# GadGadGad/Convolutional-KAN-for-Image-Classification

Hardware: AMD Instinct MI355X
Metric: images/sec fwd+bwd KAN-VGG11 3x32x32 bs=256/GPU (higher is better)
Workload: dtype f32

## Files before the change

### convolutional-kan-for-image-classification_amd/_lib.py

```python
from __future__ import annotations

import ctypes as C
import os
from typing import Optional

_HERE = os.path.dirname(os.path.abspath(__file__))
LIB_PATH = os.environ.get("KANCONV_LIB") or os.path.join(_HERE, "libkanconv.so")

KAN_MAX_PLANES = 16
KAN_MAX_TABLE = 32
KAN_FP_WORDS = 192
BASIS_BSPLINE, BASIS_RBF, BASIS_CHEBY, BASIS_POLY, BASIS_FOURIER, BASIS_RELU, BASIS_GRAM = 0, 1, 2, 3, 4, 5, 6
ACT_NONE, ACT_IDENTITY, ACT_GELU, ACT_SILU, ACT_RELU, ACT_TANH, ACT_SIGMOID, ACT_GELU_TANH = -1, 0, 1, 2, 3, 4, 5, 6


class KanGeom(C.Structure):
    _fields_ = [(n, C.c_int) for n in ("B", "C", "H", "W", "O", "Ho", "Wo", "kh", "kw", "sh", "sw", "ph", "pw", "dh", "dw", "groups")] + \
               [("x_bstride", C.c_longlong), ("y_bstride", C.c_longlong)]


class KanBasis(C.Structure):
    _fields_ = [("kind", C.c_int), ("n_basis", C.c_int), ("order", C.c_int), ("act", C.c_int),
                ("p0", C.c_float), ("p1", C.c_float), ("table", C.c_float * KAN_MAX_TABLE), ("chan_table", C.c_void_p)]


class KanPlan(C.Structure):
    _fields_ = [(n, C.c_int) for n in ("P", "K", "IPC", "KC", "Kpad", "Opad", "fwd_splits", "bwd_data_splits", "bwd_weight_splits",
                                          "fwd_target", "bwd_data_target", "bwd_weight_target", "x_pm_wanted", "dz_pm_wanted", "bwd_weight_expanded", "row_blocks", "e_pm_wanted", "fwd_expanded", "fwd_halo", "bwd_weight_halo",
# ... 11 lines not shown


class KanWavGeom(C.Structure):
    _fields_ = [(n, C.c_int) for n in ("B", "C", "H", "W", "O", "Ho", "Wo", "kh", "kw", "sh", "sw", "ph", "pw", "dh", "dw", "wavelet")] + \
               [("x_bstride", C.c_longlong), ("u_bstride", C.c_longlong)]


WAVELETS = {"mexican_hat": 0, "morlet": 1, "dog": 2, "meyer": 3, "shannon": 4}

_P, _I, _LL, _F, _D = C.c_void_p, C.c_int, C.c_longlong, C.c_float, C.c_double
_GP, _BP = C.POINTER(KanGeom), C.POINTER(KanBasis)
SIGNATURES = {
    "kan_version": (C.c_char_p, []),
    "kan_last_error": (C.c_char_p, []),
    "kan_plan": (_I, [_GP, _BP, C.POINTER(KanPlan)]),
    "kan_pack_weights": (_I, [_P, _P, _P, _P, _GP, _BP, _P]),
    "kan_pack_cacheable": (_I, [_GP, _BP]),
    "kan_pack_weights_cached": (_I, [_P, _P, _P, _P, _GP, _BP, _P, _I, _I, _I, _P]),
    "kan_conv_fwd": (_I, [_P, _P, _P, _P, _GP, _BP, _P, _P]),
    "kan_position_major": (_I, [_P, _P, _I, _I, _I, _LL, _P]),
    "kan_conv_bwd_data": (_I, [_P, _P, _P, _P, _P, _P, _GP, _BP, _P, _P]),
    "kan_conv_bwd_data_params": (_I, [_P, _P, _P, _P, _P, _P, _P, _GP, _BP, _P, _P]),
    "kan_conv_bwd_weight": (_I, [_P, _P, _P, _P, _GP, _BP, _P, _P, _P]),
    "kan_position_major_expanded": (_I, [_P, _P, _GP, _BP, _P]),
    "kan_conv_fwd_expanded": (_I, [_P, _P, _P, _GP, _BP, _P]),
    "kan_conv_bwd_weight_expanded": (_I, [_P, _P, _P, _GP, _BP, _P]),
    "kan_unpack_wgrad": (_I, [_P, _P, _P, _GP, _BP, _P]),
    "kan_slab_reduce": (_I, [_P, _I, _LL, _P, _I, _I, _I, _LL, _P]),
    "kan_instnorm_prelu_fwd": (_I, [_P, _I, _LL, _P, _P, _P, _P, _P, _P, _P, _I, _I, _I, _LL, _F, _I, _P]),
    "kan_instnorm_prelu_bwd": (_I, [_P, _P, _P, _P, _P, _P, _P, _P, _P, _P, _P, _I, _I, _I, _LL, _I, _P]),
# ... 48 lines not shown
```

### convolutional-kan-for-image-classification_amd/csrc/kan_internal.h

```cpp
#pragma once
#include <type_traits>
#include "kanconv.h"

int kan_fail_msg(const char* fmt, const char* a);
int kan_raise_lds_limit(const void* kernel, int bytes);

enum : int {
    FAST_GENERIC = 0,
    FAST_BSPLINE_SILU = 1,
    FAST_BSPLINE_GELU = 2,
    FAST_RBF8 = 3,
    FAST_CHEBY5 = 4,
    FAST_CHEBY4 = 5,
    FAST_POLY4 = 6,
    FAST_POLY3 = 7,
    FAST_RBF5 = 8,
    FAST_RELU8 = 9,
    FAST_GRAM4 = 10,
    FAST_POLY1 = 11,
    FAST_LAST = 11
};
enum : unsigned {
    ON_TAP_MAJOR = 1u << 0,
    ON_BIG_TILES = 1u << 1,
// ... 91 lines not shown

enum class Route { TAP_MAJOR, DW, BAND, HALO, EXPANDED };

struct FwdCfg { int TO, TP, tiles_o, tiles_p, chunks, splits, slots; };
struct BdCfg { int CH, tiles_c, tiles_p, n_ob, Opad32, chunks, splits; };
struct BwCfg { int TR, TO, tiles_r, tiles_o, chunks, splits, slots; };
struct BwHaloCfg { int R, nimg, spb, n_bands, tiles_r, tiles_o, splits, bands_per_split; };

struct ConvPlan {
    KanPlan pub;
    int fast;
    Route fwd, bwd_data, bwd_weight;
    bool pm_fwd, pm_bwd_data, pm_bwd_weight;
    bool rowblk_bwd_data;
    bool quad_fwd;
    bool pmdma_xcd, pm_lpt, pm_xcd;
    FwdCfg fc;
    BdCfg bd;
    BwCfg bw;
    BwHaloCfg bwh;
    KanBandCfg band;
};
int plan_conv(const KanGeom* g, const KanBasis* b, ConvPlan* cp);

int live_taps_out(const KanGeom* g, int hw);
int live_taps_in(const KanGeom* g, int hw);
int live_positions_for_tap(const KanGeom* g, int tap);
int balance_tiles(const int* weight, int n, unsigned short* idx);
```

### convolutional-kan-for-image-classification_amd/csrc/kan_plan.hip

```cpp
#include <hip/hip_runtime.h>
#include <cstdio>
#include <cstdlib>
#include <cstring>
#include "kanconv.h"
#include "kan_device.h"
#include "kan_common.h"
#include "kan_internal.h"

namespace {

int fail(const char* msg) { return kan_fail_msg("%s", msg); }

int check(const KanGeom* g, const KanBasis* b) {
    if (!g || !b) return fail("null geometry/basis");
    if (g->groups < 0 || g->groups > 65535) return fail("groups out of range");
    if (g->B <= 0 || g->C <= 0 || g->O <= 0 || g->H <= 0 || g->W <= 0 || g->Ho <= 0 || g->Wo <= 0) return fail("non-positive dimension");
    if (g->kh <= 0 || g->kw <= 0 || g->sh <= 0 || g->sw <= 0 || g->dh <= 0 || g->dw <= 0 || g->ph < 0 || g->pw < 0) return fail("bad conv parameters");
    if (g->kh > 255 || g->kw > 255 || g->C > 65535) return fail("kernel size / channel count out of supported range");
    if ((g->H + 2 * g->ph - g->dh * (g->kh - 1) - 1) / g->sh + 1 != g->Ho || (g->W + 2 * g->pw - g->dw * (g->kw - 1) - 1) / g->sw + 1 != g->Wo)
        return fail("Ho/Wo inconsistent with H/W, kernel, stride, padding, dilation");
    if ((long long)g->B * g->Ho * g->Wo >= (1ll << 31) || (long long)g->B * g->H * g->W >= (1ll << 31)) return fail("pixel count exceeds int32");
    if ((long long)g->B * g->x_bstride * 4 >= (1ll << 31) || (long long)g->B * g->y_bstride * 4 >= (1ll << 31))
        return fail("activation tensors must be smaller than 2 GiB (32-bit buffer offsets)");
    if (g->x_bstride < (long long)ngroups(g) * g->C * g->H * g->W || g->y_bstride < (long long)ngroups(g) * g->O * g->Ho * g->Wo)
// ... 324 lines not shown
    pl->bwd_weight_slab_elems = (long long)G * pl->K * pl->Opad;
    const bool big = big_tiles(f, *pl);
    c.fc = fwd_cfg(g, *pl, big, c.pm_fwd, halo);
    c.bw = bw_cfg(g, *pl, big, c.pm_bwd_weight);
    if (halo_bw) c.bwh = bw_halo_cfg(g, *pl);
    pl->fwd_splits = band ? c.band.fwd_splits : c.fc.splits;
    pl->bwd_data_splits = c.bd.splits;
    pl->bwd_weight_splits = halo_bw ? c.bwh.splits : c.bw.splits;
    if (band_bw) {
        pl->bwd_weight_splits = c.band.bw_splits;
        pl->bwd_weight_slab_elems = (long long)G * pl->Kpad * pl->Opad;
    }
    pl->fwd_target = pl->bwd_data_target = pl->bwd_weight_target = 0;
    const bool rowblk_fwd = halo && g->H == 4 && g->W == 4 && c.fc.TO == 256;
    c.quad_fwd = rowblk_fwd && g->B % 32 == 0 && !tuning_off("KAN_QUAD_FWD");
    if (dw) {
        pl->fwd_splits = pl->bwd_data_splits = 1;
        pl->bwd_weight_splits = dw_weight_chunks(g);
        pl->bwd_data_weight_bytes = pl->packed_weight_bytes;
        c.pm_fwd = c.pm_bwd_data = c.pm_bwd_weight = false;
    }
    if (c.pm_fwd) {
        LiveClass cls[16]; const int plane = g->Ho * g->Wo;
        const long long tiles_per_pos = (long long)ceil_div(g->B, c.fc.TP) * c.fc.tiles_o * G;
        for (int hw = 0; hw < plane; ++hw) cls[hw] = LiveClass{tiles_per_pos, live_taps_out(g, hw) * ceil_div(g->C, pl->IPC)};
        pl->fwd_target = pick_target_steps(cls, plane, 8, 4.0 * g->B * g->O * g->Ho * g->Wo * G, &pl->fwd_splits, c.fc.slots);
    }
    if (c.pm_bwd_weight) {
        LiveClass cw[32];
        const long long tiles_per_tap = (long long)ceil_div((long long)g->C * pl->P, c.bw.TR) * c.bw.tiles_o * G;
// ... 23 lines not shown
```

### convolutional-kan-for-image-classification_amd/csrc/kanconv.hip

```cpp
#include <hip/hip_runtime.h>
#include <cstdio>
#include <cstdlib>
#include <cstring>
#include <cmath>
#include <cstdint>
#include <mutex>
#include <type_traits>
#include <vector>
#include "kanconv.h"
#include "kan_device.h"

#include "kan_common.h"
#include "kan_internal.h"

namespace {


thread_local char g_err[512] = "";
int fail(const char* fmt, const char* a = "") {
    snprintf(g_err, sizeof(g_err), fmt, a);
    return -1;
}
}
int kan_fail_msg(const char* fmt, const char* a) { return fail(fmt, a); }
// ... 406 lines not shown
#define LDS_READ3H(r0, r1, r2, addrA, addrB, oA0, oA1, oB)                                                               \
    asm volatile("ds_read_b32 %0, %3 offset:%5\n\tds_read_b32 %1, %3 offset:%6\n\tds_read_b32 %2, %4 offset:%7"         \
                 : "=&v"(r0), "=&v"(r1), "=&v"(r2) : "v"(addrA), "v"(addrB), "n"(oA0), "n"(oA1), "n"(oB) : "memory")
#define LDS_WAIT3(r0, r1, r2, N) asm volatile("s_waitcnt lgkmcnt(" #N ")" : "+v"(r0), "+v"(r1), "+v"(r2) :: "memory")

template <int FAST, int WO, int W, int R, int NIMG, int QUAD = 0>
__global__ __launch_bounds__(WO * 2 * 64, ((WO > 2 && !(R * W == 16 && NIMG * W == 32)) ? 2 : 4)) void k_conv_fwd_halo(
    const float* __restrict__ x, const float* __restrict__ wp, float* __restrict__ z, DevGeom g, DevBasis bs, int Opad,
    int n_pairs, int pairs_per_split, long long slab_elems, unsigned x_bytes, int tiles_o) {
    constexpr int TO = WO * 64, TP = 128, NT = WO * 2 * 64, NW = WO * 2, P = fast_planes(FAST), KC = 2 * P, T = 9;
    constexpr int KIND = fast_kind(FAST);
    constexpr int HW_ = QUAD ? 3 : W + 2, HIMG = QUAD ? 9 : (R + 2) * HW_, HALO = (QUAD ? 32 : NIMG) * HIMG;
    constexpr int RPI = 256 / TO, NQ = (KC + RPI - 1) / RPI;
    static_assert(NIMG * R * W == TP && HALO % 2 == 0, "tile shape");
    static_assert(!QUAD || (R * W == 16 && NIMG * W == 32 && WO == 4), "the quadrant order is a variant of the row-block tile");
    constexpr bool ROWBLK = (R * W == 16 && NIMG * W == 32 && WO == 4) && !QUAD;
    constexpr int HPAD = QUAD ? 4 : 0;
    __shared__ __attribute__((aligned(16))) float sW[2 * KC * TO];
    __shared__ float sH_[2 * P * HALO + 2 * HPAD];
    float* const sH = sH_ + HPAD;
    __shared__ float sTab[KAN_MAX_TABLE];
    __shared__ float sDump[NT];

    const int tid = threadIdx.x, lane = tid & 63;
    const int wave = __builtin_amdgcn_readfirstlane(tid >> 6);
    const int w_o = (ROWBLK || QUAD) ? (wave & 3) : (wave >> 1), w_p = (ROWBLK || QUAD) ? (wave >> 2) : (wave & 1);
    const int HoWo = g.Ho * g.Wo, HW = g.H * g.W, Mtot = g.B * HoWo;
    const BlockId blk = xcd_block_order(true);
    const int grp = blk.y / tiles_o;
    const int qh = (blk.x >> 1) & 1, qw = blk.x & 1;
    const int px_tile0 = blk.x * TP, o_tile0 = (blk.y - grp * tiles_o) * TO;
    x += (size_t)grp * g.C * HW;
    z += (size_t)grp * g.O * HoWo;
    wp += (size_t)grp * n_pairs * (T * KC) * Opad;

    if (tid < KAN_MAX_TABLE) sTab[tid] = bs.tab[tid];
    for (int i = tid; i < 2 * P * HALO + 2 * HPAD; i += NT) sH_[i] = 0.f;

    const int b0 = QUAD ? (blk.x >> 2) * 32 : px_tile0 / HoWo, h0 = QUAD ? 0 : (px_tile0 - b0 * HoWo) / W;
    constexpr int NCELL = 2 * HALO, CPT = (NCELL + NT - 1) / NT;
    int c_src[CPT], c_dst[CPT], c_ch[CPT]; unsigned c_ok = 0;
#pragma unroll
    for (int k = 0; k < CPT; ++k) {
        const int idx = tid + k * NT;
        const int ch = idx / HALO, cell = idx - ch * HALO;
        const int img = cell / HIMG, rc = cell - img * HIMG, hr = rc / HW_, hc = rc - hr * HW_;
        const int b = b0 + img, h = QUAD ? qh + hr : h0 - 1 + hr, w = QUAD ? qw + hc : hc - 1;
        const bool ok = idx < NCELL && b < g.B && (unsigned)h < (unsigned)g.H && (unsigned)w < (unsigned)W;
        c_src[k] = b * (int)g.xbs + ch * HW + h * W + w;
        c_dst[k] = ch * (P * HALO) + cell;
        c_ch[k] = ch;
        c_ok |= (ok ? 1u : 0u) << k;
    }
    const kan_rsrc x_rs = make_rsrc(x, x_bytes);
// ... 59 lines not shown
        __syncthreads();
#pragma unroll
        for (int k = 0; k < CPT; ++k)
            if ((c_ok >> k) & 1u) stage_unit<KIND, FAST>(bs, sTab, true, xv[k], xv[k], sH + c_dst[k], HALO, sDump + tid, 2 * cp + c_ch[k]);
#pragma unroll 1
        for (int tap = 0; tap < T; ++tap) {
            asm volatile("s_waitcnt vmcnt(0)" ::: "memory");
            __syncthreads();
            const int nxt = cp * T + tap + 1;
            if (nxt < cp1 * T) issue_w(nxt, buf ^ 1);
            if (tap == 4 && cp + 1 < cp1) load_pair(cp + 1);
            const int r = tap / 3, t = tap - r * 3;
            const unsigned sh = (unsigned)(((r - 1) * HW_ + (t - 1)) * 4);
            const unsigned aw = lds_addr(sW + buf * (KC * TO) + kh2 * TO + ao), ab0 = vb[0] + sh, ab1 = vb[1] + sh;
            float fa[2][2], fb[2][2];
            const int dead = !ROWBLK ? -1 : (r == 0 && w_p == 0) ? 0 : (r == 2 && w_p == 1) ? 1 : -1;
            const bool live0 = QUAD ? ((q_live[0] >> tap) & 1u) != 0 : dead != 0, live1 = QUAD ? ((q_live[1] >> tap) & 1u) != 0 : dead != 1;
            LDS_READ4H(fa[0][0], fa[0][1], fb[0][0], fb[0][1], aw, ab0, ab1, 0, 32 * 4, 0);
#pragma unroll
            for (int kk = 0; kk < P; ++kk) {
                const int c_ = kk & 1, n_ = c_ ^ 1;
                if (kk + 1 < P) {
                    LDS_READ4H(fa[n_][0], fa[n_][1], fb[n_][0], fb[n_][1], aw, ab0, ab1, (2 * (kk + 1)) * TO * 4, (2 * (kk + 1)) * TO * 4 + 128,
                               (kk + 1) * HALO * 4);
                    LDS_WAIT4(fa[c_][0], fa[c_][1], fb[c_][0], fb[c_][1], 4);
                } else {
                    LDS_WAIT4(fa[c_][0], fa[c_][1], fb[c_][0], fb[c_][1], 0);
                }
                if (!(ROWBLK || QUAD) || live0) {
                    acc[0][0] = MFMA32(fa[c_][0], fb[c_][0], acc[0][0]);
                    acc[1][0] = MFMA32(fa[c_][1], fb[c_][0], acc[1][0]);
// ... 13 lines not shown
#pragma unroll
        for (int mi = 0; mi < 2; ++mi) {
#pragma unroll
            for (int r = 0; r < 16; ++r) {
                const int o = o_tile0 + w_o * 64 + mi * 32 + mfma_row(r, lane);
                if (o < g.O) *reinterpret_cast<float2*>(zb + (size_t)o * HoWo) = make_float2(acc[mi][0][r], acc[mi][1][r]);
            }
        }
        return;
    }
#pragma unroll
    for (int ni = 0; ni < 2; ++ni) {
        int px = px_tile0 + w_p * 64 + ni * 32 + (lane & 31);
        if (ROWBLK) {
            const int l = lane & 31;
            px = px_tile0 + (l >> 2) * (R * W) + (w_p * 2 + ni) * W + (l & 3);
        }
        if (px >= Mtot) continue;
        const int b = px / HoWo, hw = px - b * HoWo;
        float* zb = zs + (size_t)b * g.ybs + hw;
#pragma unroll
        for (int mi = 0; mi < 2; ++mi) {
#pragma unroll
            for (int r = 0; r < 16; ++r) {
                const int o = o_tile0 + w_o * 64 + mi * 32 + mfma_row(r, lane);
                if (o < g.O) zb[(size_t)o * HoWo] = acc[mi][ni][r];
            }
        }
    }
}

// ... 9 lines not shown
#pragma unroll
            for (int i = 0; i < M / 2; ++i) {
                if (i < h) {
                    const float keep = up ? v[h + i] : v[i], send = up ? v[i] : v[h + i];
                    v[i] = keep + __shfl_xor(send, off, 64);
                }
            }
            base += up ? h : 0;
            m = h;
        } else {
            v[0] += __shfl_xor(v[0], off, 64);
        }
    }
    idx = base; tot = v[0];
}

template <int KIND, int FAST, int RB = 0>
__global__ __launch_bounds__(256, 4) void k_conv_bwd_data(
    const float* __restrict__ dz, const float* __restrict__ x, const float* __restrict__ xn, const float* __restrict__ wd,
    float* __restrict__ dx, float* __restrict__ dxn, DevGeom g, DevBasis bs, int CH, int n_ct, int n_ob, int Opad16,
    int n_chunks, int chunks_per_split, long long slab_elems, unsigned dz_bytes, TilePerm perm, float* __restrict__ dpar) {
    constexpr int TP = 128, KD = 16, NT = 256;
    __shared__ __attribute__((aligned(16))) float smem[2 * 2 * KD * 128];
    __shared__ float sTab[KAN_MAX_TABLE];

    const int tid = threadIdx.x, lane = tid & 63;
    const int wave = __builtin_amdgcn_readfirstlane(tid >> 6);
    const int w_r = wave >> 1, w_p = wave & 1;
    const int HoWo = g.Ho * g.Wo, HW = g.H * g.W, P = bs.P;
    const int Min = g.B * HW;
    const BlockId blk = xcd_block_order(false);
    const int grp = blk.y / n_ct;
    const int px_tile0 = (perm.n ? (int)perm.idx[blk.x] : blk.x) * TP, ct = blk.y - grp * n_ct;
    const int ncol = n_ct * 128;
    const int pxl = (wave & 1) * 64 + lane, ol0 = wave >> 1;
    const bool idle_rows = (ct * 2 + w_r) * CH >= g.C;
    {
        const size_t xo = (size_t)grp * g.C * HW;
        x += xo; xn += xo; dx += xo; if (dxn) dxn += xo;
        dz += (size_t)grp * g.O * HoWo * (g.pix_major ? g.B : 1);
        wd += (size_t)grp * (g.kh * g.kw) * Opad16 * ncol;
    }

    if (tid < KAN_MAX_TABLE) sTab[tid] = bs.tab[tid];
    const int my_px = px_tile0 + (RB ? ((pxl >> 2) & 7) * 16 + (pxl >> 5) * 4 + (pxl & 3) : pxl);
    const bool pv = my_px < Min;
    int pb, ph_, pw_;
    {
        int hw;
        if (g.pix_major) { hw = my_px / g.B; pb = my_px - hw * g.B; }
        else { pb = my_px / HW; hw = my_px - pb * HW; }
        ph_ = hw / g.W; pw_ = hw - ph_ * g.W;
    }
    const kan_rsrc dz_rs = make_rsrc(dz, dz_bytes);
    const unsigned dz_img = g.pix_major ? (unsigned)pb : (unsigned)pb * (unsigned)g.ybs;
    const unsigned zstride = g.pix_major ? (unsigned)g.B : 1u;
    const int wv = wave;

    int cur_tap = -1; unsigned base = KAN_OOB;
    const unsigned wlane = (unsigned)((lane >> 5) * ncol + (lane & 31) * 4) * 4u;
// ... 65 lines not shown
        } else {
#pragma unroll
            for (int n = 0; n < 8; ++n)
                __builtin_amdgcn_raw_ptr_buffer_load_lds(dz_rs, (__attribute__((address_space(3))) void*)(dG + (ol0 + 2 * n) * TP), 4,
                                                         (int)baseA, (int)(soA + (unsigned)(2 * n) * row_bytes), 0, 0);
        }
        const int tapA = mixed ? t : 3 + t, tapB = 6 + t;
#pragma unroll
        for (int j = 0; j < 2; ++j) {
            const int blk2 = j * 4 + wv;
            const int row = mixed ? ((blk2 < 4 ? tapA : tapB) * Opad16 + o0 + (blk2 & 3) * 2) : (tapA * Opad16 + o0 + blk2 * 2);
            glds16((const float*)((const char*)(wd + (size_t)row * ncol + ct * 128) + wlane), dW + blk2 * 256);
        }
    };

    f32x16 acc[2][2];
#pragma unroll
    for (int a = 0; a < 2; ++a)
#pragma unroll
        for (int b = 0; b < 2; ++b)
#pragma unroll
            for (int r = 0; r < 16; ++r) acc[a][b][r] = 0.f;

    int ch0 = blk.z * chunks_per_split;
    int ch1 = min(n_chunks, ch0 + chunks_per_split);
    unsigned tapmask = 0xffffffffu;
    if (g.pix_major) {
        tapmask = 0;
        const int T = g.kh * g.kw;
        const int hwA = px_tile0 / g.B, hwB = min(px_tile0 + TP - 1, Min - 1) / g.B;
// ... 6 lines not shown
        else {
            ch0 = blk.z == 0 ? 0 : live_step_pos(tapmask, T, n_chunks, (int)((long long)L * blk.z / S), seg);
            ch1 = blk.z == S - 1 ? n_chunks : live_step_pos(tapmask, T, n_chunks, (int)((long long)L * (blk.z + 1) / S), seg);
        }
    }
    auto next_live = [&](int ch) -> int {
        if (!g.pix_major) return ch;
        while (ch < ch1) {
            const int tap = ch / n_ob;
            if ((tapmask >> tap) & 1u) return ch;
            ch = (tap + 1) * n_ob;
        }
        return ch1;
    };
    int ch = next_live(ch0);
    if (ch < ch1) { if (RB) issue_rb(ch, 0); else issue(ch, 0); }
    const int ar = w_r * 64 + (lane & 31), bp = w_p * 64 + (lane & 31), kh2 = lane >> 5;
    for (int cur = 0; ch < ch1; cur ^= 1) {
        asm volatile("s_waitcnt vmcnt(0)" ::: "memory");
        __syncthreads();
        const bool mixed_now = pend_mixed;
        ch = next_live(ch + 1);
        if (ch < ch1) { if (RB) issue_rb(ch, cur ^ 1); else issue(ch, cur ^ 1); }
        const float* cW = smem + cur * (2 * KD * 128);
        const float* cG = cW + KD * 128;
        const unsigned aw = lds_addr(cW + kh2 * 128 + ar), ag = lds_addr(cG + kh2 * TP + bp);
        if (RB) {
            const bool l0b = !(mixed_now && w_p == 0), l1a = !(mixed_now && w_p == 1);
            if (!idle_rows) KAN_MFMA_STEP_LIVE(KD / 2, aw, 128, ag, TP, true, l0b, l1a, true);
        } else if (!idle_rows) KAN_MFMA_STEP(KD / 2, aw, 128, ag, TP);
    }

    const bool same_in = (x == xn);
    const bool split_out = (dxn != nullptr);
    float* dxs = dx + (size_t)blk.z * slab_elems;
    float* dxns = split_out ? dxn + (size_t)blk.z * slab_elems : nullptr;
#define KAN_G_TO_LDS(half)                                                                                                 \
    __syncthreads();                                                                                                       \
    if (w_r == (half)) {                                                                                                   \
        _Pragma("unroll") for (int mi = 0; mi < 2; ++mi)                                                                   \
            _Pragma("unroll") for (int ni = 0; ni < 2; ++ni)                                                               \
                _Pragma("unroll") for (int r = 0; r < 16; ++r)                                                             \
// ... 1578 lines not shown
    } else if (wd) {
        const BdCfg& c = cp.bd;
        const int bx = c.tiles_c * 4, by = c.Opad32 / 32 * G;
        const long long nt = (long long)bx * by;
        const long long capd = fp ? 128 : 1024;
        dim3 gd((unsigned)(nt < capd ? nt : capd), 1, T);
        hipLaunchKernelGGL(k_pack_bwd_data, gd, dim3(256), 0, st, (const float*)wp, wd, q, c.CH, c.tiles_c, c.Opad32, wp_gs, bx, by, fp, fp_cur);
    }
    return launch_ok("pack");
}

int kan_pack_weights(const float* w_base, const float* w_basis, float* wp, float* wd, const KanGeom* g, const KanBasis* b, void* stream) {
    return pack_weights_impl(w_base, w_basis, wp, wd, g, b, nullptr, 0, stream);
}

int kan_pack_cacheable(const KanGeom* g, const KanBasis* b) {
    ConvPlan cp;
    if (plan_conv(g, b, &cp)) return 0;
    if ((long long)g->O * g->C * (b->n_basis + 1) * g->kh * g->kw >= (1ll << 31)) return 0;
    return (!pack_needs_clear(g, cp.pub) && cp.fwd != Route::DW && ngroups(g) == 1) ? 1 : 0;
}

int kan_pack_weights_cached(const float* w_base, const float* w_basis, float* wp, float* wd, const KanGeom* g, const KanBasis* b,
                            unsigned long long* ring, int cur, int force, int sample_stride, void* stream) {
    static_assert(KAN_FP_WORDS == 3 * FP_LANES, "ring size");
    if (!ring || cur < 0 || cur > 2 || sample_stride < 1) return fail("bad fingerprint ring arguments");
    if (!kan_pack_cacheable(g, b)) return fail("cached packing is not offered for this geometry (kan_pack_cacheable)");
    const int hb = b->act != KAN_ACT_NONE;
    if ((hb && !w_base) || !w_basis) return fail("null weight pointer");
    if (((size_t)w_basis & 15) || (hb && ((size_t)w_base & 15))) return fail("cached packing needs 16-byte aligned weight tensors");
// ... 66 lines not shown
        dim3 gridh(c.tiles_p, c.tiles_o * ngroups(g), pl.fwd_splits);
        dispatch_fast<ON_HALO_FWD>(cp.fast, [&](auto fv) {
            constexpr int F = decltype(fv)::value;
            auto launch = [&](auto wo, auto w, auto r, auto nimg, auto quad) {
                constexpr int WOV = decltype(wo)::value;
                hipLaunchKernelGGL((k_conv_fwd_halo<F, WOV, decltype(w)::value, decltype(r)::value, decltype(nimg)::value, decltype(quad)::value>), gridh,
                                   dim3(WOV * 128), 0, st, x, wp, z, dgh, dbh, pl.Opad, n_pairs, pps, pl.fwd_slab_elems, x_bytes, c.tiles_o);
            };
            auto planes = [&](auto wo) {
                if constexpr (decltype(wo)::value == 4) {
                    if (g->W == 4 && cp.quad_fwd && ((uintptr_t)z & 7u) == 0 && (g->y_bstride & 1) == 0 && (pl.fwd_slab_elems & 1) == 0)
                        return launch(wo, IC<4>{}, IC<4>{}, IC<8>{}, IC<1>{});
                }
                if (g->W == 32) launch(wo, IC<32>{}, IC<4>{}, IC<1>{}, IC<0>{});
                else if (g->W == 16) launch(wo, IC<16>{}, IC<8>{}, IC<1>{}, IC<0>{});
                else if (g->W == 8) launch(wo, IC<8>{}, IC<8>{}, IC<2>{}, IC<0>{});
                else launch(wo, IC<4>{}, IC<4>{}, IC<8>{}, IC<0>{});
            };
            if constexpr (fast_has(F, ON_BIG_TILES)) {
                if (c.TO == 256) return planes(IC<4>{});
            }
            planes(IC<2>{});
        });
        return launch_ok("conv_fwd_halo");
    }
    DevGeom dg = dev_geom(g);
    dg.pix_major = (x_pm && x == xn && cp.pm_fwd) ? 1 : 0;
    if (dg.pix_major) { x = x_pm; xn = x_pm; }
    DevBasis db = dev_basis(b);
    dim3 grid(c.tiles_p, c.tiles_o * ngroups(g), pl.fwd_splits);
    const int cps = dg.pix_major ? pl.fwd_target : ceil_div(c.chunks, pl.fwd_splits);
// ... 62 lines not shown
    const BdCfg& c = cp.bd;
    DevGeom dg = dev_geom(g);
    dg.pix_major = (dz_pm && cp.pm_bwd_data) ? 1 : 0;
    if (dg.pix_major) dz = dz_pm;
    DevBasis db = dev_basis(b);
    if ((long long)c.tiles_c * ngroups(g) > 65535) return fail("groups * channel tiles exceed the grid limit");
    dim3 grid(c.tiles_p, c.tiles_c * ngroups(g), pl.bwd_data_splits);
    const int cps = dg.pix_major ? pl.bwd_data_target : ceil_div(c.chunks, pl.bwd_data_splits);
    TilePerm perm; perm.n = 0;
    if (dg.pix_major) perm = tile_perm(c.tiles_p, [&](int t) {
        const int hw = (int)(((long long)t * 128) / g->B);
        return ceil_div(live_taps_in(g, hw < g->H * g->W ? hw : 0) * c.n_ob, cps > 0 ? cps : 1);
    });
    const int fast = (fast_spec(cp.fast).xn_bwd ? (x != xn && dxn) : (x == xn && !dxn)) ? cp.fast : FAST_GENERIC;
    const bool rb = !dg.pix_major && cp.rowblk_bwd_data;
    const unsigned dz_bytes = (unsigned)((long long)g->B * g->y_bstride * 4);
    auto launch = [&](auto kind, auto fast, auto rbv) {
        hipLaunchKernelGGL((k_conv_bwd_data<decltype(kind)::value, decltype(fast)::value, decltype(rbv)::value>), grid, dim3(256), 0, st, dz, x, xn, wd,
                           dx, dxn, dg, db, c.CH, c.tiles_c, c.n_ob, c.Opad32, c.chunks, cps, pl.bwd_data_slab_elems, dz_bytes, perm, dpar);
    };
    const bool launched = dispatch_fast<ON_TAP_MAJOR>(fast, [&](auto fv) {
        constexpr int F = decltype(fv)::value;
        if constexpr (fast_has(F, ON_ROWBLK_BWD_DATA)) {
            if (rb) return launch(IC<fast_kind(F)>{}, fv, IC<1>{});
        }
        launch(IC<fast_kind(F)>{}, fv, IC<0>{});
    });
    if (!launched) dispatch_kind(b->kind, [&](auto kind) { launch(kind, IC<FAST_GENERIC>{}, IC<0>{}); });
    return launch_ok("conv_bwd_data");
}

int kan_conv_bwd_weight(const float* dz, const float* x, const float* xn, float* dwp, const KanGeom* g, const KanBasis* b,
                        const float* x_pm, const float* dz_pm, void* stream) {
    ConvPlan cp;
    if (int rc = plan_conv(g, b, &cp)) return rc;
    const KanPlan& pl = cp.pub;
    if (!dz || !x || !xn || !dwp) return fail("null tensor pointer");
    if ((b->kind == KAN_BASIS_RELU || b->kind == KAN_BASIS_GRAM) && !b->chan_table) return fail("ReLU / Gram bases need their device parameter table (chan_table)");
// ... 289 lines not shown
```

### convolutional-kan-for-image-classification_amd/ops.py

```python
from __future__ import annotations

import contextlib
import ctypes as C
import os
import weakref
from collections import OrderedDict
from dataclasses import dataclass
from functools import lru_cache
from typing import List, Optional, Sequence, Tuple

import torch

from . import _lib as L


@dataclass(frozen=True)
class ConvSpec:
    kind: int
    n_basis: int
    order: int
    act: int
    p0: float
    p1: float
    table: Tuple[float, ...]
# ... 35 lines not shown
    Ho, Wo = spec.out_hw(H, W)
    if Ho <= 0 or Wo <= 0:
        raise L.KanConvError(f"empty output ({Ho}x{Wo}) for input {H}x{W}")
    g = L.KanGeom()
    g.B, g.C, g.H, g.W, g.O, g.Ho, g.Wo = B, Cg, H, W, Og, Ho, Wo
    (g.kh, g.kw), (g.sh, g.sw), (g.ph, g.pw), (g.dh, g.dw) = spec.kernel, spec.stride, spec.padding, spec.dilation
    g.x_bstride, g.y_bstride = C_total * H * W, O_total * Ho * Wo
    g.groups = spec.groups
    b = _basis_struct(spec)
    p = L.KanPlan()
    bp = b
    if _device_table(spec):
        bp = L.KanBasis.from_buffer_copy(b)
        bp.chan_table = 1
    L.check(L.load().kan_plan(C.byref(g), C.byref(bp), C.byref(p)), "kan_plan")
    return g, b, p


def _plan_key(spec: ConvSpec, shape, Og: int) -> tuple:
    B, Ct, H, W = shape
    return (spec, B, Ct // spec.groups, H, W, Og, Ct, Og * spec.groups)


def _with_phases(basis: L.KanBasis, phases: Optional[torch.Tensor], mode: int = 0) -> L.KanBasis:
    if phases is None:
        return basis
    b = L.KanBasis.from_buffer_copy(basis)
    b.chan_table, b.order = phases.data_ptr(), mode
    return b

# ... 75 lines not shown
        for wo in range(Wo):
            for r in range(kh):
                for t in range(kw):
                    hi, wi = ho * sh - ph + r * dh, wo * sw - pw + t * dw
                    live += 0 <= hi < H and 0 <= wi < W
    return live / float(Ho * Wo * kh * kw)


_ROW_BLOCK_BIT = {"fwd": 1, "bwd_data": 2, "bwd_weight": 0}


def _quadrant_order(geom, plan, which: str) -> bool:
    return which == "fwd" and bool(plan.row_blocks & 1) and geom.B % 32 == 0


def _executed_flops(geom, plan, which: str) -> float:
    target = {"fwd": plan.fwd_target, "bwd_data": plan.bwd_data_target, "bwd_weight": plan.bwd_weight_target}[which]
    dense = _conv_flops(geom, plan)
    g = geom
    if target <= 0:
        if _quadrant_order(geom, plan, which):
            return dense * _live_fraction(which, g.H, g.W, g.Ho, g.Wo, g.kh, g.kw, g.sh, g.sw, g.ph, g.pw, g.dh, g.dw)
        if plan.row_blocks & _ROW_BLOCK_BIT[which]:
            return dense * (5.0 / 6.0)
        return dense
    return dense * _live_fraction(which, g.H, g.W, g.Ho, g.Wo, g.kh, g.kw, g.sh, g.sw, g.ph, g.pw, g.dh, g.dw)


def _layer_tag(geom) -> str:
    return f"{geom.C * max(1, geom.groups)}->{geom.O * max(1, geom.groups)}@{geom.H}x{geom.W} k{geom.kh}x{geom.kw}"


def _sample(which: str, geom, plan, pm: bool, two: bool = False, expanded: bool = False):
    tile = "128" if plan.Opad % 128 == 0 else "64"
    if which == "bwd_data":
        name = "k_conv_bwd_data"
    elif expanded:
        name = f"k_conv_{which}_pmdma/o{tile}"
    elif plan.fwd_band if which == "fwd" else plan.bwd_weight_band:
        name = f"k_band_{which}/o" + ("128" if plan.Opad % 128 == 0 else "192" if plan.Opad == 192 else "64")
    else:
        halo = plan.fwd_halo if which == "fwd" else (plan.bwd_weight_halo and not two)
        name = f"k_conv_{which}{'_halo' if halo else ''}/o{tile}"
    skips = expanded or pm or bool(plan.row_blocks & _ROW_BLOCK_BIT[which])
    dense = _conv_flops(geom, plan)
    return name, dense, _executed_flops(geom, plan, which) if skips else dense, _layer_tag(geom)


def _position_major(t: torch.Tensor, ch_off: int, Cn: int) -> torch.Tensor:
    B, Ct, H, W = t.shape
    out = torch.empty(Cn * H * W * B, device=t.device, dtype=torch.float32)
    L.check(L.load().kan_position_major(_ptr(t, ch_off * H * W), _ptr(out), B, Cn, H * W, Ct * H * W, _stream(t)), "kan_position_major")
    return out


def _stack(ws: Sequence[Optional[torch.Tensor]]) -> Optional[torch.Tensor]:
    if ws[0] is None:
        return None
    return ws[0].unsqueeze(0) if len(ws) == 1 else torch.stack(list(ws))


# ... 579 lines not shown
```

### include/kanconv.h

```cpp
#ifndef KANCONV_H
#define KANCONV_H

#ifdef __cplusplus
extern "C" {
#endif

#define KAN_MAX_PLANES 16
#define KAN_MAX_TABLE  32
#define KAN_FP_WORDS   192

enum { KAN_BASIS_BSPLINE = 0, KAN_BASIS_RBF = 1, KAN_BASIS_CHEBY = 2, KAN_BASIS_POLY = 3, KAN_BASIS_FOURIER = 4, KAN_BASIS_RELU = 5, KAN_BASIS_GRAM = 6 };
enum { KAN_ACT_NONE = -1, KAN_ACT_IDENTITY = 0, KAN_ACT_GELU = 1, KAN_ACT_SILU = 2, KAN_ACT_RELU = 3,
       KAN_ACT_TANH = 4, KAN_ACT_SIGMOID = 5, KAN_ACT_GELU_TANH = 6 };

typedef struct KanGeom {
    int B, C, H, W;
    int O, Ho, Wo;
    int kh, kw, sh, sw, ph, pw, dh, dw;
    int groups;
    long long x_bstride;
    long long y_bstride;
} KanGeom;

#define KAN_ORDER_PACK(mode, first) ((int)(mode) | ((int)(first) << 8))
// ... 21 lines not shown
    int e_pm_wanted, fwd_expanded;
    int fwd_halo, bwd_weight_halo;
    int fwd_band, bwd_weight_band;
    long long packed_weight_bytes;
    long long bwd_data_weight_bytes;
    long long fwd_slab_elems;
    long long bwd_data_slab_elems;
    long long bwd_weight_slab_elems;
    long long e_pm_elems;
} KanPlan;

const char* kan_version(void);
const char* kan_last_error(void);

int kan_plan(const KanGeom* geom, const KanBasis* basis, KanPlan* plan);

int kan_pack_weights(const float* w_base, const float* w_basis, float* wp, float* wd,
                     const KanGeom* geom, const KanBasis* basis, void* stream);

int kan_pack_cacheable(const KanGeom* geom, const KanBasis* basis);
int kan_pack_weights_cached(const float* w_base, const float* w_basis, float* wp, float* wd,
                            const KanGeom* geom, const KanBasis* basis, unsigned long long* ring, int cur, int force,
                            int sample_stride, void* stream);

int kan_conv_fwd(const float* x, const float* xn, const float* wp, float* z,
                 const KanGeom* geom, const KanBasis* basis, const float* x_pm, void* stream);

int kan_position_major(const float* src, float* dst, int B, int Cn, int HW, long long bstride, void* stream);

int kan_conv_bwd_data(const float* dz, const float* x, const float* xn, const float* wd,
// ... 87 lines not shown
```

Measured before the change: 17530.

## Add quadrant tile order for bwd-data and row-block tiles for 8x8 forward

```diff
diff --git a/convolutional-kan-for-image-classification_amd/_lib.py b/convolutional-kan-for-image-classification_amd/_lib.py
--- a/convolutional-kan-for-image-classification_amd/_lib.py
+++ b/convolutional-kan-for-image-classification_amd/_lib.py
@@ -12,6 +12,7 @@
 KAN_FP_WORDS = 192
 BASIS_BSPLINE, BASIS_RBF, BASIS_CHEBY, BASIS_POLY, BASIS_FOURIER, BASIS_RELU, BASIS_GRAM = 0, 1, 2, 3, 4, 5, 6
 ACT_NONE, ACT_IDENTITY, ACT_GELU, ACT_SILU, ACT_RELU, ACT_TANH, ACT_SIGMOID, ACT_GELU_TANH = -1, 0, 1, 2, 3, 4, 5, 6
+ORDER_QUAD_FWD, ORDER_ROWBLK8_FWD, ORDER_QUAD_BWD_DATA = 1, 2, 4
 
 
 class KanGeom(C.Structure):
@@ -53,6 +54,7 @@
     "kan_version": (C.c_char_p, []),
     "kan_last_error": (C.c_char_p, []),
     "kan_plan": (_I, [_GP, _BP, C.POINTER(KanPlan)]),
+    "kan_tile_orders": (_I, [_GP, _BP]),
     "kan_pack_weights": (_I, [_P, _P, _P, _P, _GP, _BP, _P]),
     "kan_pack_cacheable": (_I, [_GP, _BP]),
     "kan_pack_weights_cached": (_I, [_P, _P, _P, _P, _GP, _BP, _P, _I, _I, _I, _P]),
diff --git a/convolutional-kan-for-image-classification_amd/csrc/kan_internal.h b/convolutional-kan-for-image-classification_amd/csrc/kan_internal.h
--- a/convolutional-kan-for-image-classification_amd/csrc/kan_internal.h
+++ b/convolutional-kan-for-image-classification_amd/csrc/kan_internal.h
@@ -129,6 +129,8 @@
     bool pm_fwd, pm_bwd_data, pm_bwd_weight;
     bool rowblk_bwd_data;
     bool quad_fwd;
+    bool quad_bd;
+    bool rowblk8_fwd;
     bool pmdma_xcd, pm_lpt, pm_xcd;
     FwdCfg fc;
     BdCfg bd;
diff --git a/convolutional-kan-for-image-classification_amd/csrc/kan_plan.hip b/convolutional-kan-for-image-classification_amd/csrc/kan_plan.hip
--- a/convolutional-kan-for-image-classification_amd/csrc/kan_plan.hip
+++ b/convolutional-kan-for-image-classification_amd/csrc/kan_plan.hip
@@ -362,6 +362,8 @@
     pl->fwd_target = pl->bwd_data_target = pl->bwd_weight_target = 0;
     const bool rowblk_fwd = halo && g->H == 4 && g->W == 4 && c.fc.TO == 256;
     c.quad_fwd = rowblk_fwd && g->B % 32 == 0 && !tuning_off("KAN_QUAD_FWD");
+    c.quad_bd = c.rowblk_bwd_data && g->B % 32 == 0 && !tuning_off("KAN_QUAD_BD");
+    c.rowblk8_fwd = halo && g->H == 8 && g->W == 8 && c.fc.TO == 256 && g->B % 4 == 0 && !tuning_off("KAN_ROWBLK8_FWD");
     if (dw) {
         pl->fwd_splits = pl->bwd_data_splits = 1;
         pl->bwd_weight_splits = dw_weight_chunks(g);
diff --git a/convolutional-kan-for-image-classification_amd/csrc/kanconv.hip b/convolutional-kan-for-image-classification_amd/csrc/kanconv.hip
--- a/convolutional-kan-for-image-classification_amd/csrc/kanconv.hip
+++ b/convolutional-kan-for-image-classification_amd/csrc/kanconv.hip
@@ -444,7 +444,8 @@
     constexpr int RPI = 256 / TO, NQ = (KC + RPI - 1) / RPI;
     static_assert(NIMG * R * W == TP && HALO % 2 == 0, "tile shape");
     static_assert(!QUAD || (R * W == 16 && NIMG * W == 32 && WO == 4), "the quadrant order is a variant of the row-block tile");
-    constexpr bool ROWBLK = (R * W == 16 && NIMG * W == 32 && WO == 4) && !QUAD;
+    constexpr bool ROWBLK = (NIMG * W == 32 && R == 4 && WO == 4) && !QUAD;
+    constexpr bool HALFPL = ROWBLK && W == 8;
     constexpr int HPAD = QUAD ? 4 : 0;
     __shared__ __attribute__((aligned(16))) float sW[2 * KC * TO];
     __shared__ float sH_[2 * P * HALO + 2 * HPAD];
@@ -467,7 +468,8 @@
     if (tid < KAN_MAX_TABLE) sTab[tid] = bs.tab[tid];
     for (int i = tid; i < 2 * P * HALO + 2 * HPAD; i += NT) sH_[i] = 0.f;
 
-    const int b0 = QUAD ? (blk.x >> 2) * 32 : px_tile0 / HoWo, h0 = QUAD ? 0 : (px_tile0 - b0 * HoWo) / W;
+    const int b0 = QUAD ? (blk.x >> 2) * 32 : HALFPL ? (blk.x >> 1) * NIMG : px_tile0 / HoWo;
+    const int h0 = QUAD ? 0 : HALFPL ? (blk.x & 1) * R : (px_tile0 - b0 * HoWo) / W;
     constexpr int NCELL = 2 * HALO, CPT = (NCELL + NT - 1) / NT;
     int c_src[CPT], c_dst[CPT], c_ch[CPT]; unsigned c_ok = 0;
 #pragma unroll
@@ -557,7 +559,7 @@
             const unsigned sh = (unsigned)(((r - 1) * HW_ + (t - 1)) * 4);
             const unsigned aw = lds_addr(sW + buf * (KC * TO) + kh2 * TO + ao), ab0 = vb[0] + sh, ab1 = vb[1] + sh;
             float fa[2][2], fb[2][2];
-            const int dead = !ROWBLK ? -1 : (r == 0 && w_p == 0) ? 0 : (r == 2 && w_p == 1) ? 1 : -1;
+            const int dead = !ROWBLK ? -1 : (r == 0 && w_p == 0 && h0 == 0) ? 0 : (r == 2 && w_p == 1 && h0 + R == g.H) ? 1 : -1;
             const bool live0 = QUAD ? ((q_live[0] >> tap) & 1u) != 0 : dead != 0, live1 = QUAD ? ((q_live[1] >> tap) & 1u) != 0 : dead != 1;
             LDS_READ4H(fa[0][0], fa[0][1], fb[0][0], fb[0][1], aw, ab0, ab1, 0, 32 * 4, 0);
 #pragma unroll
@@ -601,7 +603,7 @@
         int px = px_tile0 + w_p * 64 + ni * 32 + (lane & 31);
         if (ROWBLK) {
             const int l = lane & 31;
-            px = px_tile0 + (l >> 2) * (R * W) + (w_p * 2 + ni) * W + (l & 3);
+            px = (b0 + l / W) * HoWo + (h0 + w_p * 2 + ni) * W + l % W;
         }
         if (px >= Mtot) continue;
         const int b = px / HoWo, hw = px - b * HoWo;
@@ -641,6 +643,30 @@
     }
     idx = base; tot = v[0];
 }
+
+#define KAN_MFMA_STEP_QUAD(NK, addrA, LDA, addrB, l0, l1)                                                                           \
+    do {                                                                                                                           \
+        float fa_[2][2], fb_[2][2];                                                                                                \
+        LDS_READ4(fa_[0][0], fa_[0][1], fb_[0][0], fb_[0][1], addrA, addrB, 0, 32 * 4, 0, 512 * 4);                                \
+        _Pragma("unroll") for (int kk = 0; kk < (NK); ++kk) {                                                                       \
+            const int c_ = kk & 1, n_ = c_ ^ 1;                                                                                    \
+            if (kk + 1 < (NK)) {                                                                                                   \
+                LDS_READ4(fa_[n_][0], fa_[n_][1], fb_[n_][0], fb_[n_][1], addrA, addrB, (2 * (kk + 1)) * (LDA) * 4,                \
+                          (2 * (kk + 1)) * (LDA) * 4 + 128, (2 * (kk + 1)) * 32 * 4, (2 * (kk + 1)) * 32 * 4 + 512 * 4);           \
+                LDS_WAIT4(fa_[c_][0], fa_[c_][1], fb_[c_][0], fb_[c_][1], 4);                                                      \
+            } else {                                                                                                               \
+                LDS_WAIT4(fa_[c_][0], fa_[c_][1], fb_[c_][0], fb_[c_][1], 0);                                                      \
+            }                                                                                                                      \
+            if (l0) {                                                                                                              \
+                acc[0][0] = MFMA32(fa_[c_][0], fb_[c_][0], acc[0][0]);                                                             \
+                acc[1][0] = MFMA32(fa_[c_][1], fb_[c_][0], acc[1][0]);                                                             \
+            }                                                                                                                      \
+            if (l1) {                                                                                                              \
+                acc[0][1] = MFMA32(fa_[c_][0], fb_[c_][1], acc[0][1]);                                                             \
+                acc[1][1] = MFMA32(fa_[c_][1], fb_[c_][1], acc[1][1]);                                                             \
+            }                                                                                                                      \
+        }                                                                                                                          \
+    } while (0)
 
 template <int KIND, int FAST, int RB = 0>
 __global__ __launch_bounds__(256, 4) void k_conv_bwd_data(
@@ -665,12 +691,23 @@
     {
         const size_t xo = (size_t)grp * g.C * HW;
         x += xo; xn += xo; dx += xo; if (dxn) dxn += xo;
-        dz += (size_t)grp * g.O * HoWo * (g.pix_major ? g.B : 1);
+        dz += (size_t)grp * g.O * HoWo * ((g.pix_major || RB == 2) ? g.B : 1);
         wd += (size_t)grp * (g.kh * g.kw) * Opad16 * ncol;
     }
 
     if (tid < KAN_MAX_TABLE) sTab[tid] = bs.tab[tid];
-    const int my_px = px_tile0 + (RB ? ((pxl >> 2) & 7) * 16 + (pxl >> 5) * 4 + (pxl & 3) : pxl);
+    const int q_qh = (blk.x >> 1) & 1, q_qw = blk.x & 1, q_b0 = (blk.x >> 2) * 32;
+    auto q_pos = [&](int bk) { return ((bk == 0 || bk == 2) ? 3 * q_qh : 1 + q_qh) * 4 + ((bk == 0 || bk == 3) ? 3 * q_qw : 1 + q_qw); };
+    auto q_mask = [&](int hw) {
+        unsigned m = 0;
+        for (int tap = 0; tap < 9; ++tap) {
+            const int r = tap / 3, t = tap - r * 3;
+            m |= (((unsigned)((hw >> 2) + 1 - r) < 4u && (unsigned)((hw & 3) + 1 - t) < 4u) ? 1u : 0u) << tap;
+        }
+        return m;
+    };
+    const int my_px = RB == 2 ? (q_b0 + (pxl & 31)) * 16 + q_pos(pxl >> 5)
+                              : px_tile0 + (RB == 1 ? ((pxl >> 2) & 7) * 16 + (pxl >> 5) * 4 + (pxl & 3) : pxl);
     const bool pv = my_px < Min;
     int pb, ph_, pw_;
     {
@@ -766,6 +803,30 @@
         }
     };
 
+    const int cp_hw = q_pos(wv); const unsigned cp_live = q_mask(cp_hw);
+    const unsigned q_live0 = q_mask(q_pos(2 * w_p)), q_live1 = q_mask(q_pos(2 * w_p + 1));
+    const unsigned q_voff = (unsigned)((lane >> 3) * 16 * g.B + (lane & 7) * 4) * 4u;
+    int pend_tap = 0;
+    auto issue_q = [&](int ch, int buf) {
+        const int tap = ch / n_ob, o0 = (ch - tap * n_ob) * KD;
+        pend_tap = tap;
+        float* dW = smem + buf * (2 * KD * 128);
+        float* dG = dW + KD * 128 + wv * 512;
+        if ((cp_live >> tap) & 1u) {
+            const int r = tap / 3, t = tap - r * 3;
+            const unsigned so = (unsigned)((o0 * 16 + cp_hw + (1 - r) * 4 + (1 - t)) * g.B + q_b0) * 4u;
+            __builtin_amdgcn_raw_ptr_buffer_load_lds(dz_rs, (__attribute__((address_space(3))) void*)dG, 16, (int)q_voff, (int)so, 0, 0);
+            __builtin_amdgcn_raw_ptr_buffer_load_lds(dz_rs, (__attribute__((address_space(3))) void*)(dG + 256), 16, (int)q_voff,
+                                                     (int)(so + (unsigned)(8 * 16 * g.B) * 4u), 0, 0);
+        }
+        const char* wsrc = (const char*)(wd + ((size_t)tap * Opad16 + o0) * ncol + ct * 128);
+#pragma unroll
+        for (int j = 0; j < 2; ++j) {
+            const int blk2 = j * 4 + wv;
+            glds16((const float*)(wsrc + (size_t)blk2 * 2 * ncol * 4 + wlane), dW + blk2 * 256);
+        }
+    };
+
     f32x16 acc[2][2];
 #pragma unroll
     for (int a = 0; a < 2; ++a)
@@ -802,18 +863,23 @@
         return ch1;
     };
     int ch = next_live(ch0);
-    if (ch < ch1) { if (RB) issue_rb(ch, 0); else issue(ch, 0); }
+    if (ch < ch1) { if (RB == 2) issue_q(ch, 0); else if (RB) issue_rb(ch, 0); else issue(ch, 0); }
     const int ar = w_r * 64 + (lane & 31), bp = w_p * 64 + (lane & 31), kh2 = lane >> 5;
     for (int cur = 0; ch < ch1; cur ^= 1) {
         asm volatile("s_waitcnt vmcnt(0)" ::: "memory");
         __syncthreads();
         const bool mixed_now = pend_mixed;
+        const int tap_now = pend_tap;
         ch = next_live(ch + 1);
-        if (ch < ch1) { if (RB) issue_rb(ch, cur ^ 1); else issue(ch, cur ^ 1); }
+        if (ch < ch1) { if (RB == 2) issue_q(ch, cur ^ 1); else if (RB) issue_rb(ch, cur ^ 1); else issue(ch, cur ^ 1); }
         const float* cW = smem + cur * (2 * KD * 128);
         const float* cG = cW + KD * 128;
         const unsigned aw = lds_addr(cW + kh2 * 128 + ar), ag = lds_addr(cG + kh2 * TP + bp);
-        if (RB) {
+        if (RB == 2) {
+            const unsigned agq = lds_addr(cG + (2 * w_p) * 512 + kh2 * 32 + (lane & 31));
+            const bool l0 = ((q_live0 >> tap_now) & 1u) != 0, l1 = ((q_live1 >> tap_now) & 1u) != 0;
+            if (!idle_rows) KAN_MFMA_STEP_QUAD(KD / 2, aw, 128, agq, l0, l1);
+        } else if (RB) {
             const bool l0b = !(mixed_now && w_p == 0), l1a = !(mixed_now && w_p == 1);
             if (!idle_rows) KAN_MFMA_STEP_LIVE(KD / 2, aw, 128, ag, TP, true, l0b, l1a, true);
         } else if (!idle_rows) KAN_MFMA_STEP(KD / 2, aw, 128, ag, TP);
@@ -2422,6 +2488,13 @@
     return pack_weights_impl(w_base, w_basis, wp, wd, g, b, nullptr, 0, stream);
 }
 
+int kan_tile_orders(const KanGeom* g, const KanBasis* b) {
+    ConvPlan cp;
+    if (plan_conv(g, b, &cp)) return 0;
+    const bool halo = cp.fwd == Route::HALO;
+    return (halo && cp.quad_fwd ? KAN_ORDER_QUAD_FWD : 0) | (halo && cp.rowblk8_fwd ? KAN_ORDER_ROWBLK8_FWD : 0) | (cp.quad_bd ? KAN_ORDER_QUAD_BWD_DATA : 0);
+}
+
 int kan_pack_cacheable(const KanGeom* g, const KanBasis* b) {
     ConvPlan cp;
     if (plan_conv(g, b, &cp)) return 0;
@@ -2518,7 +2591,12 @@
                 }
                 if (g->W == 32) launch(wo, IC<32>{}, IC<4>{}, IC<1>{}, IC<0>{});
                 else if (g->W == 16) launch(wo, IC<16>{}, IC<8>{}, IC<1>{}, IC<0>{});
-                else if (g->W == 8) launch(wo, IC<8>{}, IC<8>{}, IC<2>{}, IC<0>{});
+                else if (g->W == 8) {
+                    if constexpr (decltype(wo)::value == 4) {
+                        if (cp.rowblk8_fwd) return launch(wo, IC<8>{}, IC<4>{}, IC<4>{}, IC<0>{});
+                    }
+                    launch(wo, IC<8>{}, IC<8>{}, IC<2>{}, IC<0>{});
+                }
                 else launch(wo, IC<4>{}, IC<4>{}, IC<8>{}, IC<0>{});
             };
             if constexpr (fast_has(F, ON_BIG_TILES)) {
@@ -2611,14 +2689,17 @@
     });
     const int fast = (fast_spec(cp.fast).xn_bwd ? (x != xn && dxn) : (x == xn && !dxn)) ? cp.fast : FAST_GENERIC;
     const bool rb = !dg.pix_major && cp.rowblk_bwd_data;
+    const bool quad = rb && cp.quad_bd && dz_pm && x == xn && !dxn;
     const unsigned dz_bytes = (unsigned)((long long)g->B * g->y_bstride * 4);
     auto launch = [&](auto kind, auto fast, auto rbv) {
-        hipLaunchKernelGGL((k_conv_bwd_data<decltype(kind)::value, decltype(fast)::value, decltype(rbv)::value>), grid, dim3(256), 0, st, dz, x, xn, wd,
+        hipLaunchKernelGGL((k_conv_bwd_data<decltype(kind)::value, decltype(fast)::value, decltype(rbv)::value>), grid, dim3(256), 0, st,
+                           decltype(rbv)::value == 2 ? dz_pm : dz, x, xn, wd,
                            dx, dxn, dg, db, c.CH, c.tiles_c, c.n_ob, c.Opad32, c.chunks, cps, pl.bwd_data_slab_elems, dz_bytes, perm, dpar);
     };
     const bool launched = dispatch_fast<ON_TAP_MAJOR>(fast, [&](auto fv) {
         constexpr int F = decltype(fv)::value;
         if constexpr (fast_has(F, ON_ROWBLK_BWD_DATA)) {
+            if (quad) return launch(IC<fast_kind(F)>{}, fv, IC<2>{});
             if (rb) return launch(IC<fast_kind(F)>{}, fv, IC<1>{});
         }
         launch(IC<fast_kind(F)>{}, fv, IC<0>{});
diff --git a/convolutional-kan-for-image-classification_amd/ops.py b/convolutional-kan-for-image-classification_amd/ops.py
--- a/convolutional-kan-for-image-classification_amd/ops.py
+++ b/convolutional-kan-for-image-classification_amd/ops.py
@@ -73,6 +73,7 @@
         bp = L.KanBasis.from_buffer_copy(b)
         bp.chan_table = 1
     L.check(L.load().kan_plan(C.byref(g), C.byref(bp), C.byref(p)), "kan_plan")
+    p.tile_orders = L.load().kan_tile_orders(C.byref(g), C.byref(bp))
     return g, b, p
 
 
@@ -178,15 +179,25 @@
     return which == "fwd" and bool(plan.row_blocks & 1) and geom.B % 32 == 0
 
 
-def _executed_flops(geom, plan, which: str) -> float:
+def _quadrant_bwd_data(geom, plan, have_dz_pm: bool) -> bool:
+    return bool(have_dz_pm) and bool(plan.row_blocks & 2) and bool(getattr(plan, "tile_orders", 0) & L.ORDER_QUAD_BWD_DATA)
+
+
+def _row_blocks8_forward(geom, plan) -> bool:
+    return geom.H == 8 and geom.W == 8 and bool(getattr(plan, "tile_orders", 0) & L.ORDER_ROWBLK8_FWD)
+
+
+def _executed_flops(geom, plan, which: str, have_dz_pm: bool = False) -> float:
     target = {"fwd": plan.fwd_target, "bwd_data": plan.bwd_data_target, "bwd_weight": plan.bwd_weight_target}[which]
     dense = _conv_flops(geom, plan)
     g = geom
     if target <= 0:
-        if _quadrant_order(geom, plan, which):
+        if _quadrant_order(geom, plan, which) or (which == "bwd_data" and _quadrant_bwd_data(geom, plan, have_dz_pm)):
             return dense * _live_fraction(which, g.H, g.W, g.Ho, g.Wo, g.kh, g.kw, g.sh, g.sw, g.ph, g.pw, g.dh, g.dw)
         if plan.row_blocks & _ROW_BLOCK_BIT[which]:
             return dense * (5.0 / 6.0)
+        if which == "fwd" and _row_blocks8_forward(geom, plan):
+            return dense * (11.0 / 12.0)
         return dense
     return dense * _live_fraction(which, g.H, g.W, g.Ho, g.Wo, g.kh, g.kw, g.sh, g.sw, g.ph, g.pw, g.dh, g.dw)
 
@@ -206,9 +217,9 @@
     else:
         halo = plan.fwd_halo if which == "fwd" else (plan.bwd_weight_halo and not two)
         name = f"k_conv_{which}{'_halo' if halo else ''}/o{tile}"
-    skips = expanded or pm or bool(plan.row_blocks & _ROW_BLOCK_BIT[which])
+    skips = expanded or pm or bool(plan.row_blocks & _ROW_BLOCK_BIT[which]) or (which == "fwd" and _row_blocks8_forward(geom, plan))
     dense = _conv_flops(geom, plan)
-    return name, dense, _executed_flops(geom, plan, which) if skips else dense, _layer_tag(geom)
+    return name, dense, _executed_flops(geom, plan, which, pm) if skips else dense, _layer_tag(geom)
 
 
 def _position_major(t: torch.Tensor, ch_off: int, Cn: int) -> torch.Tensor:
diff --git a/include/kanconv.h b/include/kanconv.h
--- a/include/kanconv.h
+++ b/include/kanconv.h
@@ -59,6 +59,11 @@
 const char* kan_last_error(void);
 
 int kan_plan(const KanGeom* geom, const KanBasis* basis, KanPlan* plan);
+
+#define KAN_ORDER_QUAD_FWD 1
+#define KAN_ORDER_ROWBLK8_FWD 2
+#define KAN_ORDER_QUAD_BWD_DATA 4
+int kan_tile_orders(const KanGeom* geom, const KanBasis* basis);
 
 int kan_pack_weights(const float* w_base, const float* w_basis, float* wp, float* wd,
                      const KanGeom* geom, const KanBasis* basis, void* stream);
```

Result: faster. 17870, median of 6 (+1.9%).
